# NoelShin/zutis

Hardware: AMD Instinct MI355X
Metric: images/sec, COCO2017-val-shaped ViT-B/16 dense semantic segmentation @336px (ZUTIS forward + semantic predict), batches of 32 per GPU, 3 independent batches in flight (higher is better)
Workload: dtype f16x3 (fp32-class)

## Files before the change

### include/zutis_hip.h

```cpp
#ifndef ZUTIS_HIP_H
#define ZUTIS_HIP_H

#include <stddef.h>

#ifdef __cplusplus
extern "C" {
#endif

typedef struct ihipStream_t* zh_stream_t;

#define ZH_OK 0
#define ZH_ERR_ARG (-1)
#define ZH_ERR_HIP (-2)
#define ZH_ERR_WORKSPACE (-3)

#define ZH_ACT_NONE 0
#define ZH_ACT_QUICKGELU 1
#define ZH_ACT_RELU 2
#define ZH_ACT_SIGMOID 3
#define ZH_ACT_GELU_ERF 4

#define ZH_ABI_VERSION 232
int zh_version(void);
const char* zh_arch(void);
const char* zh_last_error(void);

int zh_dev_set_gemm_overrides(int group_m, int tile, int tile_small);

int zh_dev_set_gemm_persist(int workgroups);

int zh_gemm_f16(const void* A, long lda, long strideA, const void* W, long ldw, long strideW,
                void* C, long ldc, long strideC, int out_f16,
                const float* bias, const float* residual, long ldr, long strideR, int res_rows,
                const void* pos_y, const void* pos_x, long ld_pos, int pos_h, int pos_w, int pos_f16,
                int act, int M, int N, int K, int batch, zh_stream_t stream);

int zh_gemm_f16_res16(const void* A, long lda, long strideA, const void* W, long ldw, long strideW,
// ... 41 lines not shown
                     const float* add, int add_rows, int rows, int D, long lo_plane, int* status, zh_stream_t stream);
#define ZH_STATUS_RANGE 1
#define ZH_STATUS_NONFINITE 2
#define ZH_STATUS_LABEL 4

int zh_sum_layernorm_f32(const float* parts, int n_parts, long part_stride, const float* bias, const float* residual,
                         float* out_sum, const float* gamma, const float* beta, float eps,
                         float* out_f32, void* out_f16, long lo_plane,
                         long out_group_rows, long out_group_stride, long out_offset, int skip_first_in_group,
                         const float* gamma2, const float* beta2, float eps2, float* out2_f32, void* out2_f16, long lo_plane2,
                         long out2_group_rows, long out2_group_stride, long out2_offset,
                         int rows, int D, int* status, zh_stream_t stream);

int zh_assemble_tokens_ln(const float* patch_emb, const float* class_embedding, const float* pos_embed,
                          const float* gamma, const float* beta, float eps, float* out,
                          int B, int T, int D, zh_stream_t stream);

int zh_assemble_tokens_ln_f16(const float* patch_emb, const float* class_embedding, const float* pos_embed,
                              const float* gamma, const float* beta, float eps, void* out,
                              int B, int T, int D, zh_stream_t stream);

int zh_l2norm_rows(const float* x, float* out_f32, void* out_f16, float eps, int rows, int D, long lo_plane, float f16_scale, zh_stream_t stream);

size_t zh_global_ln_l2_workspace_size(int B, int M, int C);
int zh_global_ln_l2(const float* x, float* out_f32, void* out_f16, float eps, float l2_eps,
                    int B, int M, int C, void* workspace, size_t workspace_bytes, long lo_plane, float f16_scale, int* status,
                    zh_stream_t stream);

int zh_im2col_f16(const float* x, void* out, int B, int Cin, int H, int W, int patch, int Kpad, int pad_to_patch,
                  long lo_plane, zh_stream_t stream);

int zh_posembed_bicubic(const float* pos, float* out, int grid, int h, int w, int D, float scale_h, float scale_w,
                        int has_cls, zh_stream_t stream);

int zh_upsample2x_bilinear_cl(const float* x, float* out_f32, void* out_f16, int B, int h, int w, int D, long lo_plane,
                              int relu, zh_stream_t stream);

int zh_sine_pe(float* out, int h, int w, int D, float temperature, zh_stream_t stream);

int zh_add_rowperiodic_f16(const void* a, const float* add, void* out, long rows, int D, int add_rows, long a_lo_plane,
                           long lo_plane, zh_stream_t stream);

// ... 136 lines not shown
```

### zutis_amd/csrc/common.h

```cpp
#pragma once
#include <hip/hip_runtime.h>
#include <stdint.h>
#include <stdio.h>

typedef _Float16 half_t;
typedef _Float16 half2_t __attribute__((ext_vector_type(2)));
typedef _Float16 half4_t __attribute__((ext_vector_type(4)));
typedef _Float16 half8_t __attribute__((ext_vector_type(8)));
typedef float f32x4 __attribute__((ext_vector_type(4)));
typedef float f32x16 __attribute__((ext_vector_type(16)));

#define ZH_OK 0
#define ZH_ERR_ARG (-1)
#define ZH_ERR_HIP (-2)
#define ZH_ERR_WORKSPACE (-3)

void zh_set_error(const char* fmt, ...);

#define ZH_CHECK_ARG(cond, ...)            \
  do {                                     \
    if (!(cond)) {                         \
      zh_set_error(__VA_ARGS__);           \
      return ZH_ERR_ARG;                   \
    }                                      \
// ... 55 lines not shown
  if (lo_plane) p[lo_plane] = (half_t)(y - (float)h);
}

struct LinW { int i0, i1; float l0, l1; };
__device__ __forceinline__ LinW lin_weights(int dst, int in_size, int out_size, float scale) {
  LinW r;
  if (in_size == out_size) { r.i0 = r.i1 = dst; r.l0 = 1.f; r.l1 = 0.f; return r; }
  const float src = fmaxf(__fmaf_rn(scale, (float)dst + 0.5f, -0.5f), 0.f);
  r.i0 = min((int)src, in_size - 1);
  r.i1 = min(r.i0 + 1, in_size - 1);
  r.l1 = fminf(fmaxf(src - (float)r.i0, 0.f), 1.f);
  r.l0 = 1.f - r.l1;
  return r;
}

#define ZH_ACT_NONE 0
#define ZH_ACT_QUICKGELU 1
#define ZH_ACT_RELU 2
#define ZH_ACT_SIGMOID 3
#define ZH_ACT_GELU_ERF 4

__device__ __forceinline__ float zh_act(float x, int act) {
  switch (act) {
    case ZH_ACT_QUICKGELU: return x * __builtin_amdgcn_rcpf(1.0f + __expf(-1.702f * x));
    case ZH_ACT_RELU: return fmaxf(x, 0.0f);
    case ZH_ACT_SIGMOID: return __builtin_amdgcn_rcpf(1.0f + __expf(-x));
    case ZH_ACT_GELU_ERF: return 0.5f * x * (1.0f + erff(x * 0.70710678118654752f));
    default: return x;
  }
}
// ... 1 lines not shown
```

### zutis_amd/csrc/norm.hip

```cpp
#include "common.h"

#define LN_MAXV 4

struct LnRow {
  f32x4 v[LN_MAXV];
};

#define ZH_STATUS_NONFINITE 2

__device__ __forceinline__ bool ln_normalize(LnRow& r, int nv, int lane, int D, float eps) {
  float s = 0.f;
#pragma unroll
  for (int j = 0; j < LN_MAXV; ++j)
    if (lane + 64 * j < nv) s += (r.v[j][0] + r.v[j][1]) + (r.v[j][2] + r.v[j][3]);
  const float mean = wave_sum(s) / (float)D;
  float q = 0.f;
#pragma unroll
  for (int j = 0; j < LN_MAXV; ++j)
    if (lane + 64 * j < nv) {
      r.v[j] -= mean;
      q += (r.v[j][0] * r.v[j][0] + r.v[j][1] * r.v[j][1]) + (r.v[j][2] * r.v[j][2] + r.v[j][3] * r.v[j][3]);
    }
  const float var = wave_sum(q) / (float)D;
  const float rstd = rsqrtf(var + eps);
// ... 186 lines not shown
  SumLnArgs p{parts, n_parts, part_stride, bias, residual, out_sum, gamma, beta, eps, out_f32, (half_t*)out_f16, lo_plane,
              out_group_rows, out_group_stride, out_offset, skip_first_in_group, gamma2, beta2, eps2, out2_f32, (half_t*)out2_f16, lo_plane2,
              out2_group_rows, out2_group_stride, out2_offset, rows, D, status};
  const dim3 grid(zh_cdiv(rows, 4));
  if (n_parts == 1) hipLaunchKernelGGL(sum_layernorm_kernel<1>, grid, dim3(256), 0, stream, p);
  else if (n_parts == 2) hipLaunchKernelGGL(sum_layernorm_kernel<2>, grid, dim3(256), 0, stream, p);
  else if (n_parts == 4) hipLaunchKernelGGL(sum_layernorm_kernel<4>, grid, dim3(256), 0, stream, p);
  else hipLaunchKernelGGL(sum_layernorm_kernel<0>, grid, dim3(256), 0, stream, p);
  ZH_CHECK_LAUNCH("zh_sum_layernorm_f32");
  return ZH_OK;
}

struct AsmArgs {
  const float* patch; const float* cls; const float* pos; const float* gamma; const float* beta;
  float* out; int B, T, D; float eps;
};

__global__ __launch_bounds__(256) void assemble_ln_kernel(AsmArgs p) {
  const int lane = threadIdx.x & 63;
  const long r = (long)blockIdx.x * 4 + (threadIdx.x >> 6);
  if (r >= (long)p.B * p.T) return;
  const int nv = p.D >> 2;
  const int b = (int)(r / p.T), t = (int)(r % p.T);
  const f32x4* src = t == 0 ? (const f32x4*)p.cls : (const f32x4*)(p.patch + ((long)b * (p.T - 1) + (t - 1)) * p.D);
  const f32x4* pos = (const f32x4*)(p.pos + (long)t * p.D);
  LnRow row;
#pragma unroll
  for (int j = 0; j < LN_MAXV; ++j)
    if (lane + 64 * j < nv) row.v[j] = src[lane + 64 * j] + pos[lane + 64 * j];
  if (p.gamma) ln_normalize(row, nv, lane, p.D, p.eps);
#pragma unroll
  for (int j = 0; j < LN_MAXV; ++j) {
    const int c = lane + 64 * j;
    if (c < nv) ((f32x4*)(p.out + r * p.D))[c] = p.gamma ? row.v[j] * ((const f32x4*)p.gamma)[c] + ((const f32x4*)p.beta)[c] : row.v[j];
  }
}

extern "C" int zh_assemble_tokens_ln(const float* patch_emb, const float* class_embedding, const float* pos_embed,
                                     const float* gamma, const float* beta, float eps, float* out,
                                     int B, int T, int D, hipStream_t stream) {
  ZH_CHECK_ARG(patch_emb && class_embedding && pos_embed && out, "zh_assemble_tokens_ln: null pointer");
  ZH_CHECK_ARG((gamma == nullptr) == (beta == nullptr), "zh_assemble_tokens_ln: gamma and beta must both be given or both null");
  ZH_CHECK_ARG(B > 0 && T > 1 && D % 4 == 0 && D <= 256 * LN_MAXV, "zh_assemble_tokens_ln: bad shape B=%d T=%d D=%d", B, T, D);
  AsmArgs p{patch_emb, class_embedding, pos_embed, gamma, beta, out, B, T, D, eps};
  hipLaunchKernelGGL(assemble_ln_kernel, dim3(zh_cdiv((long)B * T, 4)), dim3(256), 0, stream, p);
  ZH_CHECK_LAUNCH("zh_assemble_tokens_ln");
  return ZH_OK;
}

__device__ __forceinline__ bool ln_normalize_h8(LnRow& r, int nv8, int lane, int D, float eps) {
  float s = 0.f;
#pragma unroll
  for (int j = 0; j < LN_MAXV; ++j)
    if (lane + 64 * (j >> 1) < nv8) s += (r.v[j][0] + r.v[j][1]) + (r.v[j][2] + r.v[j][3]);
  const float mean = wave_sum(s) / (float)D;
  float q = 0.f;
#pragma unroll
  for (int j = 0; j < LN_MAXV; ++j)
    if (lane + 64 * (j >> 1) < nv8) {
// ... 88 lines not shown
  if (p.gamma) ln_normalize(row, nv, lane, p.D, p.eps);
  half_t* out = (half_t*)(void*)p.out + r * p.D;
#pragma unroll
  for (int j = 0; j < LN_MAXV; ++j) {
    const int c = lane + 64 * j;
    if (c < nv) zh_store_h4(out + 4 * c, 0, p.gamma ? row.v[j] * ((const f32x4*)p.gamma)[c] + ((const f32x4*)p.beta)[c] : row.v[j]);
  }
}

extern "C" int zh_assemble_tokens_ln_f16(const float* patch_emb, const float* class_embedding, const float* pos_embed,
                                         const float* gamma, const float* beta, float eps, void* out,
                                         int B, int T, int D, hipStream_t stream) {
  ZH_CHECK_ARG(patch_emb && class_embedding && pos_embed && out, "zh_assemble_tokens_ln_f16: null pointer");
  ZH_CHECK_ARG((gamma == nullptr) == (beta == nullptr), "zh_assemble_tokens_ln_f16: gamma and beta must both be given or both null");
  ZH_CHECK_ARG(B > 0 && T > 1 && D % 4 == 0 && D <= 256 * LN_MAXV, "zh_assemble_tokens_ln_f16: bad shape B=%d T=%d D=%d", B, T, D);
  AsmArgs p{patch_emb, class_embedding, pos_embed, gamma, beta, (float*)out, B, T, D, eps};
  hipLaunchKernelGGL(assemble_ln_h16_kernel, dim3(zh_cdiv((long)B * T, 4)), dim3(256), 0, stream, p);
  ZH_CHECK_LAUNCH("zh_assemble_tokens_ln_f16");
  return ZH_OK;
}

__global__ __launch_bounds__(256) void l2norm_rows_kernel(const float* x, float* out_f32, half_t* out_f16, int rows, int D, float eps,
                                                          long lo_plane, float f16_scale) {
  const int lane = threadIdx.x & 63;
  const long r = (long)blockIdx.x * 4 + (threadIdx.x >> 6);
  if (r >= rows) return;
  const int nv = D >> 2;
  const f32x4* xp = (const f32x4*)(x + r * D);
  f32x4 v[LN_MAXV];
  float q = 0.f;
#pragma unroll
// ... 99 lines not shown
#pragma unroll
  for (int j = 0; j < LN_MAXV; ++j)
    if (lane + 64 * j < nv) {
      v[j] = (xp[lane + 64 * j] - fmean) * rstd;
      q += (v[j][0] * v[j][0] + v[j][1] * v[j][1]) + (v[j][2] * v[j][2] + v[j][3] * v[j][3]);
    }
  const float inv = 1.0f / (sqrtf(wave_sum(q)) + l2_eps);
  const long ob = (long)img * per_image + r * C;
#pragma unroll
  for (int j = 0; j < LN_MAXV; ++j) {
    const int c = lane + 64 * j;
    if (c < nv) {
      f32x4 y = v[j] * inv;
      if (out_f32) ((f32x4*)(out_f32 + ob))[c] = y;
      if (out_f16) zh_store_h4(out_f16 + ob + 4 * c, lo_plane, y * f16_scale);
    }
  }
}

extern "C" size_t zh_global_ln_l2_workspace_size(int B, int M, int C) {
  const long per_image = (long)M * C;
  return (size_t)B * zh_cdiv(per_image, GLN_CHUNK) * 4 * sizeof(float);
}

extern "C" int zh_global_ln_l2(const float* x, float* out_f32, void* out_f16, float eps, float l2_eps,
                               int B, int M, int C, void* workspace, size_t workspace_bytes, long lo_plane, float f16_scale, int* status,
                               hipStream_t stream) {
  ZH_CHECK_ARG(x && (out_f32 || out_f16) && B > 0 && M > 0 && lo_plane % 4 == 0 && f16_scale > 0.f, "zh_global_ln_l2: bad arguments");
  ZH_CHECK_ARG(C % 4 == 0 && C <= 256 * LN_MAXV && C > 0, "zh_global_ln_l2: C=%d unsupported", C);
  ZH_CHECK_ARG(B < 65536, "zh_global_ln_l2: batch too large");
  const long per_image = (long)M * C;
  const int nchunks = zh_cdiv(per_image, GLN_CHUNK);
  if (workspace_bytes < zh_global_ln_l2_workspace_size(B, M, C) || !workspace) {
    zh_set_error("zh_global_ln_l2: workspace too small (%zu < %zu)", workspace_bytes, zh_global_ln_l2_workspace_size(B, M, C));
    return ZH_ERR_WORKSPACE;
  }
  hipLaunchKernelGGL(gln_partial_kernel, dim3(nchunks, B), dim3(256), 0, stream, x, (float*)workspace, per_image, nchunks);
  hipLaunchKernelGGL(gln_apply_kernel, dim3(zh_cdiv(M, 4), B), dim3(256), 0, stream, x, (const float*)workspace, out_f32,
                     (half_t*)out_f16, per_image, nchunks, M, C, eps, l2_eps, lo_plane, f16_scale, status);
  ZH_CHECK_LAUNCH("zh_global_ln_l2");
  return ZH_OK;
}
```

### zutis_amd/csrc/resample.hip

```cpp
#include "common.h"

__global__ __launch_bounds__(128) void im2col_kernel(const float* x, half_t* out, int B, int Cin, int H, int W, int p,
                                                     int gh, int gw, int Kpad, int vec, long lo_plane) {
  const int row = blockIdx.x;
  const int px = row % gw;
  const int t = row / gw;
  const int py = t % gh, b = t / gh;
  const int pp = p * p, kreal = Cin * pp;
  half_t* orow = out + (long)row * Kpad;
  for (int k0 = threadIdx.x * 8; k0 < Kpad; k0 += 128 * 8) {
    half8_t o;
    if (vec && k0 + 8 <= kreal) {
      const int c = k0 / pp, ij = k0 - c * pp, i = ij / p, j = ij - i * p;
      const int yy = py * p + i, xx = px * p + j;
      if (yy < H && xx + 8 <= W) {
        const f32x4* src = (const f32x4*)(x + (((long)b * Cin + c) * H + yy) * W + xx);
        const f32x4 v0 = src[0], v1 = src[1];
        zh_store_h4(orow + k0, lo_plane, v0);
        zh_store_h4(orow + k0 + 4, lo_plane, v1);
        continue;
      }
    }
#pragma unroll
    for (int e = 0; e < 8; ++e) {
// ... 93 lines not shown
  const int ya = max(j, 0), yb = min(j + 1, h - 1), xa = max(k, 0), xc = min(k + 1, w - 1);
  const f32x4* xb = (const f32x4*)(x + (long)b * h * w * D);
  const f32x4* p00 = xb + (long)(ya * w + xa) * nv;
  const f32x4* p01 = xb + (long)(ya * w + xc) * nv;
  const f32x4* p10 = xb + (long)(yb * w + xa) * nv;
  const f32x4* p11 = xb + (long)(yb * w + xc) * nv;
  float ly1[2], lx1[2];
  long orow[2];
  int ocol[2];
  bool vy[2], vx[2];
#pragma unroll
  for (int s = 0; s < 2; ++s) {
    const int oy = 2 * j + 1 + s, ox = 2 * k + 1 + s;
    vy[s] = oy >= 0 && oy < 2 * h;
    vx[s] = ox >= 0 && ox < 2 * w;
    const float sy = fmaxf(__fmaf_rn(0.5f, (float)oy + 0.5f, -0.5f), 0.f), sx = fmaxf(__fmaf_rn(0.5f, (float)ox + 0.5f, -0.5f), 0.f);
    const int y0 = min((int)sy, h - 1), x0 = min((int)sx, w - 1);
    ly1[s] = fminf(fmaxf(sy - (float)y0, 0.f), 1.f);
    lx1[s] = fminf(fmaxf(sx - (float)x0, 0.f), 1.f);
    orow[s] = ((long)b * 2 * h + oy) * (2 * w);
    ocol[s] = ox;
  }
  for (int c = threadIdx.x; c < nv; c += blockDim.x) {
    const f32x4 v00 = p00[c], v01 = p01[c], v10 = p10[c], v11 = p11[c];
#pragma unroll
    for (int sy = 0; sy < 2; ++sy)
#pragma unroll
      for (int sx = 0; sx < 2; ++sx) {
        if (!(vy[sy] && vx[sx])) continue;
        const float lx0 = 1.f - lx1[sx], ly0 = 1.f - ly1[sy];
        f32x4 o;
#pragma unroll
        for (int e = 0; e < 4; ++e) {
          const float r0 = __fmaf_rn(v00[e], lx0, __fmul_rn(v01[e], lx1[sx]));
          const float r1 = __fmaf_rn(v10[e], lx0, __fmul_rn(v11[e], lx1[sx]));
          o[e] = __fmaf_rn(r0, ly0, __fmul_rn(r1, ly1[sy]));
          if (relu) o[e] = fmaxf(o[e], 0.0f);
        }
        const long oi = (orow[sy] + ocol[sx]) * nv + c;
        if (out_f32) ((f32x4*)out_f32)[oi] = o;
        if (out_f16) zh_store_h4(out_f16 + 4 * oi, lo_plane, o);
      }
  }
}

extern "C" int zh_upsample2x_bilinear_cl(const float* x, float* out_f32, void* out_f16, int B, int h, int w, int D, long lo_plane,
                                         int relu, hipStream_t stream) {
  ZH_CHECK_ARG(x && (out_f32 || out_f16) && B > 0 && h > 0 && w > 0 && D > 0 && D % 4 == 0 && lo_plane % 4 == 0,
               "zh_upsample2x_bilinear_cl: bad arguments");
  const long quads = (long)B * (h + 1) * (w + 1);
  ZH_CHECK_ARG(quads < (1L << 31), "zh_upsample2x_bilinear_cl: too many output quads");
// ... 530 lines not shown
```

### zutis_amd/engine.py

```python
from __future__ import annotations

import math
import weakref
from typing import Dict, Optional, Tuple

import numpy as np
import torch

from . import _lib, compose, ops
from ._lib import ZutisHipError
from .engine_base import (ALL_SITES, DECODER_SITES, ENCODER_SITES, HEAD_SITES, PRECISIONS, P_shape0, _EngineBase, _rup, f16, f32,
                          resolve_precision)
from .ops import Act


def _to_host(t: torch.Tensor, cache: Dict[int, torch.Tensor]) -> np.ndarray:
    n = t.numel()
    if cache is None:
        cache = {}
    buf = cache.get(n)
    if buf is None:
        while len(cache) >= 8:
            cache.pop(next(iter(cache)))
        buf = cache[n] = torch.empty((n,), dtype=torch.uint8, pin_memory=True)
    buf.copy_(t, non_blocking=True)
    torch.cuda.current_stream(t.device).synchronize()
    return buf.numpy()


class ZutisEngine(_EngineBase):

    def __init__(self, params: Dict[str, torch.Tensor], patch: int, dec_heads: int = 8, precision="exact"):
        self.params = params
        self.patch = patch
        self.D = params["encoder.class_embedding"].shape[0]
        self.heads = self.D // 64
        self.layers = 1 + max(int(k.split(".")[3]) for k in params if k.startswith("encoder.transformer.resblocks."))
        self.dec_layers = 1 + max(int(k.split(".")[2]) for k in params if k.startswith("decoder.layers."))
        self.dec_heads = dec_heads
        self.dec_dh = self.D // dec_heads
        self.Q = params["query_embed"].shape[0]
        self.E = params["encoder.proj"].shape[1]
        self.grid = int(math.isqrt(params["encoder.positional_embedding"].shape[0] - 1))
        if self.dec_dh not in (64, 96):
            raise ZutisHipError(f"decoder head_dim {self.dec_dh} unsupported by zh_attention_f16 (64 or 96)")
        self._init_base(precision)

    def _pack(self):
        key = self._version_key()
        if key == self._packed_key:
            return
        P, D, w = self.params, self.D, {}
        c32 = self._c32
        self._pack_clip_visual(w, P, "encoder.", D, self.layers, self.patch)
        for ffn in ("ffn1", "ffn2"):
            for j in range(3):
                if (ffn, j) == ("ffn1", 2):
                    continue
                w[f"{ffn}.{j}.w"], w[f"{ffn}.{j}.b"] = self._hw(P[f"{ffn}.layers.{j}.weight"], ffn), c32(P[f"{ffn}.layers.{j}.bias"])
        W2, b2 = P["ffn1.layers.2.weight"].detach(), P["ffn1.layers.2.bias"].detach()
        self.Fh = W2.shape[1]
# ... 65 lines not shown
        g1 = self._abuf("ffn2_h1", (RQ, Fh), self._x3("ffn2"))
        g2 = self._abuf("ffn2_h2", (RQ, Fh), self._x3("ffn2"))
        q32 = self._buf("q32", (RQ, D), f32)
        q16 = self._abuf("q16", (RQ, D), self._x3("mask"), unit_norm=True)
        self._gemm("ffn2", inter16, W_["ffn2.0.w"], g1, bias=W_["ffn2.0.b"], act=ops.ACT_RELU)
        self._gemm("ffn2", g1, W_["ffn2.1.w"], g2, bias=W_["ffn2.1.b"], act=ops.ACT_RELU)
        self._gemm("ffn2", g2, W_["ffn2.2.w"], q32, bias=W_["ffn2.2.b"])
        ops.l2norm_rows(q32, RQ, D, out_f16=q16)
        masks = torch.empty((B, L, Q, h2, w2), dtype=f32, device=x.device)
        qw = self._abuf("mask_q", (RQ, FX), self._x3("mask"))
        self._gemm("mask", q16, W_["mask_q.w"], qw)
        self._gemm("mask", qw, f2x, masks, act=ops.ACT_SIGMOID, M=L * Q, N=M, K=FX, lda=FX, ldw=FX, ldc=M,
                   batch=B, strideA=L * Q * FX, strideW=M * FX, strideC=L * Q * M)
        tsl = self._buf("textspace_lo", (B * h * w, self.E), f32)
        self._gemm("textproj", tok16, W_["projT"], tsl)
        ts = self._buf("textspace", (B * M, self.E), f32)
        ops.upsample2x_cl(tsl, B, h, w, self.E, out_f32=ts)
        pt = torch.empty((B, h2, w2, self.E), dtype=f32, device=x.device)
        ws = self._buf("gln_ws", (max(1, ops.global_ln_l2_workspace_size(B, M, self.E)),), torch.uint8)
        pt16 = self._abuf("pt16", (B * M, self.E), self._x3("logits"), unit_norm=True)
        ops.global_ln_l2(ts, B, M, self.E, out_f32=pt, out_f16=pt16, eps=1e-5, l2_eps=1e-7, workspace=ws, status=self.status_word())
        self._pt16_of = (weakref.ref(pt), pt._version)
        return {"mask_proposals": masks, "patch_tokens": pt}

    def forward_graphed(self, x: torch.Tensor) -> Dict[str, torch.Tensor]:
        key = tuple(x.shape)
        graphs = self._graphs
        g = graphs.get(key)
        if g is not None and g["weights"] is self._packed_key:
            graphs.move_to_end(key)
            if g["graph"] is None:
                return self.forward(x)
            g["x"].copy_(x)
            g["graph"].replay()
            out = {k: v.clone() for k, v in g["out"].items()}
            if self._version_key() == self._packed_key:
# ... 306 lines not shown
```

### zutis_amd/engine_base.py

```python
from __future__ import annotations

import collections

import math
import os
import weakref
from typing import Dict, Optional, Tuple

import numpy as np
import torch

from . import _lib, compose, ops
from ._lib import ZutisHipError

from .ops import Act


def P_shape0(w) -> int:
    return (w.hi if isinstance(w, Act) else w).shape[0]

f16, f32 = torch.float16, torch.float32

ENCODER_SITES = ("conv", "qkv", "attn", "out", "fc", "proj")
DECODER_SITES = ("dec_kv", "dec")
# ... 70 lines not shown

    def _init_base(self, precision="exact", allow_half: bool = False):
        self.x3_sites = resolve_precision(precision, allow_half)
        self.precision = precision if isinstance(precision, str) else "custom"
        self.half_stream = precision == HALF
        self._packed_key = None
        self._w: Dict[str, torch.Tensor] = {}
        self._geo: Dict[Tuple[int, int], Dict[str, torch.Tensor]] = {}
        self._graphs: "collections.OrderedDict" = collections.OrderedDict()
        self._bufs: Dict[Tuple, torch.Tensor] = {}
        self._pinned: Dict[int, torch.Tensor] = {}
        self._buf_gen = 0
        self._buf_const: Dict[str, torch.Tensor] = {}
        self._pt16_of = self._text16_of = None
        self._status = None

    def fork(self):
        import copy
        self._pack()
        e = copy.copy(self)
        e._bufs, e._buf_gen, e._buf_const = {}, 0, {}
        e._geo = dict(self._geo)
        e._graphs = collections.OrderedDict()
        e._pinned = {}
        e._pt16_of = e._text16_of = None
        e._status = None
        return e

    def status_word(self) -> torch.Tensor:
        if self._status is None:
# ... 121 lines not shown
            w[q + "out_w"], w[q + "out_b"] = hw(P[p + "attn.out_proj.weight"], "out"), c32(P[p + "attn.out_proj.bias"])
            w[q + "fc_w"], w[q + "fc_b"] = hw(P[p + "mlp.c_fc.weight"], "fc"), c32(P[p + "mlp.c_fc.bias"])
            w[q + "proj_w"], w[q + "proj_b"] = hw(P[p + "mlp.c_proj.weight"], "proj"), c32(P[p + "mlp.c_proj.bias"])
            for ln, ln2 in (("ln_1", "ln1"), ("ln_2", "ln2")):
                w[q + ln2 + ".w"], w[q + ln2 + ".b"] = c32(P[p + ln + ".weight"]), c32(P[p + ln + ".bias"])

    def _clip_trunk(self, x: torch.Tensor, pos: torch.Tensor, h: int, w: int):
        W_, D, p = self._w, self.D, self.patch
        B = x.shape[0]
        T, R = 1 + h * w, B * (1 + h * w)
        col = self._abuf("col", (B * h * w, self.Kc), self._x3("conv"))
        ops.im2col(x, col, p, self.Kc)
        pe32 = self._buf("patch_emb", (B * h * w, D), f32)
        self._gemm("conv", col, W_["conv"], pe32)
        X = self._buf("X", (R, D), f16 if self.half_stream else f32)
        ops.assemble_tokens_ln(pe32, W_["encoder.class_embedding"], pos, W_["encoder.ln_pre.weight"],
                               W_["encoder.ln_pre.bias"], 1e-5, X, B, T, D)
        self._vit_blocks(X, B, T, D, self.heads, self.layers, 1e-5, ops.ACT_QUICKGELU)
        return X

    def _vit_blocks(self, X, B, T, D, heads, n_layers, eps, act, causal=False):
        W_, R = self._w, B * T
        Fd = P_shape0(W_["enc.0.fc_w"])
        Y = self._abuf("Y16", (R, D), self._x3("qkv", "fc"))
        xa = self._x3("attn")
        QKV = self._abuf("QKV16", (R, 3 * D), xa)
        O = self._abuf("O16", (R, D), self._x3("out"))
        Hh = self._abuf("H16", (R, Fd), self._x3("proj"))
        q_, k_, v_ = QKV, QKV.view(QKV.hi[:, D:]), QKV.view(QKV.hi[:, 2 * D:])
        st = self.status_word()
        s_out, s_proj = self._splitk(R, D, D), self._splitk(R, D, Fd)
        sk = self._x3("out") and self._x3("proj") and (s_out > 1 or s_proj > 1)
        if X.dtype == f16 and (self._x3("out") or self._x3("proj")):
            raise ZutisHipError("an fp16 residual stream needs the fp16-operand out / proj GEMMs (precision \"half\")")
        parts = self._buf("sk_parts", (max(s_out, s_proj), R, D), f32) if sk else None

# ... 1 lines not shown
            K = A.hi.shape[-1]
            return self._gemm(site, A, Wt, parts, M=R, N=D, K=K // S, lda=K, ldw=K, ldc=D, batch=S, strideA=K // S, strideW=K // S, strideC=R * D)
        eks, ews = 1, None
        if not causal:
            per_image = heads * -(-T // 128)
            eks = max(1, min(8, 256 // per_image)) if B * per_image <= 128 else 1
            ktiles = -(-T // (32 if xa else 64))
            if eks == 1 and T >= 2048:
                eks = long_sequence_key_split(B * per_image, ktiles, D // heads, xa, B * T * D)
            while eks > 1 and (eks - 1) * -(-ktiles // eks) >= ktiles:
                eks -= 1
            if eks > 1:
                ews = self._buf("enc_attn_ws", (ops.attention_splitk_workspace_size(B, heads, T, D // heads, eks),), torch.uint8)
        for i in range(n_layers):
            pp = f"enc.{i}."
            if not (sk and s_proj > 1 and i > 0):
                ops.layernorm(X, W_[pp + "ln1.w"], W_[pp + "ln1.b"], eps, R, D, out_f16=Y, status=st)
            self._gemm("qkv", Y, W_[pp + "qkv_w"], QKV, bias=W_[pp + "qkv_b"])
            ops.attention(q_, k_, v_, O, batch=B, heads=heads, Tq=T, Tk=T, head_dim=D // heads,
                          ldq=3 * D, ldk=3 * D, ldv=3 * D, ldo=D, strideQ=T * 3 * D, strideK=T * 3 * D, strideV=T * 3 * D,
                          strideO=T * D, causal=causal, x3=xa, ksplit=eks, workspace=ews)
            if sk and s_out > 1:
                gemm_parts("out", O, W_[pp + "out_w"], s_out)
                ops.sum_layernorm(parts, s_out, R, D, bias=W_[pp + "out_b"], residual=X, out_sum=X, gamma=W_[pp + "ln2.w"], beta=W_[pp + "ln2.b"],
                                  eps=eps, out_f16=Y, status=st)
            else:
                self._gemm("out", O, W_[pp + "out_w"], X, bias=W_[pp + "out_b"], residual=X)
                ops.layernorm(X, W_[pp + "ln2.w"], W_[pp + "ln2.b"], eps, R, D, out_f16=Y, status=st)
            self._gemm("fc", Y, W_[pp + "fc_w"], Hh, bias=W_[pp + "fc_b"], act=act)
            if sk and s_proj > 1:
                gemm_parts("proj", Hh, W_[pp + "proj_w"], s_proj)
# ... 107 lines not shown
```

### zutis_amd/ops.py

```python
from __future__ import annotations

import math
from typing import Optional

import numpy as np
import torch

from . import _lib

ACT_NONE, ACT_QUICKGELU, ACT_RELU, ACT_SIGMOID, ACT_GELU_ERF = 0, 1, 2, 3, 4
f16, f32 = torch.float16, torch.float32


PROFILER = None


def _call(entry: str, *args):
    _lib.check(getattr(_lib.load(), entry)(*args), entry)


def _launch(name, work, entry: str, args):
    fn = getattr(_lib.load(), entry)
    _lib.check(fn(*args) if PROFILER is None else PROFILER(name, work, lambda: fn(*args)), entry)

# ... 241 lines not shown
                  out_f32=None, out_f16=None, out_group_rows=None, out_group_stride=None, out_offset=0, skip_first_in_group=False,
                  gamma2=None, beta2=None, eps2=1e-5, out2_f32=None, out2_f16=None, out2_group_rows=None, out2_group_stride=None, out2_offset=0,
                  status=None):
    part_stride = rows * D if part_stride is None else part_stride
    ogr = rows if out_group_rows is None else out_group_rows
    ogs = ogr if out_group_stride is None else out_group_stride
    ogr2 = rows if out2_group_rows is None else out2_group_rows
    ogs2 = ogr2 if out2_group_stride is None else out2_group_stride
    (out_f16, lo1), (out2_f16, lo2) = _hp(out_f16), _hp(out2_f16)
    _call("zh_sum_layernorm_f32", _p(parts), n_parts, part_stride, _p(bias), _p(residual), _p(out_sum), _p(gamma), _p(beta), float(eps),
          _p(out_f32), _p(out_f16), lo1, ogr, ogs, out_offset, int(skip_first_in_group),
          _p(gamma2), _p(beta2), float(eps2), _p(out2_f32), _p(out2_f16), lo2, ogr2, ogs2, out2_offset,
          rows, D, _p(status), _stream())


def assemble_tokens_ln(patch_emb, cls, pos, gamma, beta, eps, out, B, T, D):
    _call("zh_assemble_tokens_ln_f16" if out.dtype == f16 else "zh_assemble_tokens_ln", _p(patch_emb), _p(cls), _p(pos), _p(gamma), _p(beta),
          float(eps), _p(out), B, T, D, _stream())


def _f16_scale(a) -> float:
    return 1.0 / a.out_scale if isinstance(a, Act) else 1.0


def l2norm_rows(x, rows, D, out_f32=None, out_f16=None, eps=0.0):
    sc = _f16_scale(out_f16)
    out_f16, lo = _hp(out_f16)
    _call("zh_l2norm_rows", _p(x), _p(out_f32), _p(out_f16), float(eps), rows, D, lo, sc, _stream())


def global_ln_l2_workspace_size(B, M, Cc) -> int:
    return int(_lib.load(raw=True).zh_global_ln_l2_workspace_size(B, M, Cc))


def global_ln_l2(x, B, M, Cc, out_f32=None, out_f16=None, eps=1e-5, l2_eps=1e-7, workspace=None, status=None):
    need = global_ln_l2_workspace_size(B, M, Cc)
    if workspace is None or _nbytes(workspace) < need:
        workspace = torch.empty(need, dtype=torch.uint8, device=x.device)
    sc = _f16_scale(out_f16)
    out_f16, lo = _hp(out_f16)
    _call("zh_global_ln_l2", _p(x), _p(out_f32), _p(out_f16), float(eps), float(l2_eps), B, M, Cc, _p(workspace),
          _nbytes(workspace), lo, sc, _p(status), _stream())


def im2col(x, out, patch, Kpad, pad_to_patch=False):
    B, Cin, H, W = x.shape
    _chk(x, f32, "im2col x")
    out, lo = _hp(out)
    _call("zh_im2col_f16", _p(x), _p(out), B, Cin, H, W, patch, Kpad, int(pad_to_patch), lo, _stream())


def posembed_bicubic(pos, out, grid, h, w, D, scale_h, scale_w, has_cls=True):
    _call("zh_posembed_bicubic", _p(pos), _p(out), grid, h, w, D, float(np.float32(scale_h)), float(np.float32(scale_w)), int(has_cls), _stream())


def upsample2x_cl(x, B, h, w, D, out_f32=None, out_f16=None, relu=False):
# ... 464 lines not shown
```

Before: 3076.

## Fuse upsample into global LN+L2 and chain first-block LayerNorm into token assembly

Adds a kernel pair that recomputes the 2x bilinear upsample on the fly inside the global LayerNorm+L2 normalisation. The full-resolution fp32 textspace buffer is no longer written and read back. Separately, the token-assembly ln_pre kernel now also applies the first encoder block's ln1 and writes the f16 (hi/lo) operand, skipping one layernorm launch and one pass over X. The fused path recomputes the interpolation in both the partial-stats and apply passes, and it changes the reduction structure, which could slightly alter numerics.

```diff
diff --git a/include/zutis_hip.h b/include/zutis_hip.h
--- a/include/zutis_hip.h
+++ b/include/zutis_hip.h
@@ -20,7 +20,7 @@
 #define ZH_ACT_SIGMOID 3
 #define ZH_ACT_GELU_ERF 4
 
-#define ZH_ABI_VERSION 232
+#define ZH_ABI_VERSION 233
 int zh_version(void);
 const char* zh_arch(void);
 const char* zh_last_error(void);
@@ -92,6 +92,7 @@
 
 int zh_assemble_tokens_ln(const float* patch_emb, const float* class_embedding, const float* pos_embed,
                           const float* gamma, const float* beta, float eps, float* out,
+                          const float* gamma2, const float* beta2, float eps2, void* out2_f16, long lo_plane2, int* status,
                           int B, int T, int D, zh_stream_t stream);
 
 int zh_assemble_tokens_ln_f16(const float* patch_emb, const float* class_embedding, const float* pos_embed,
@@ -104,6 +105,10 @@
 int zh_global_ln_l2(const float* x, float* out_f32, void* out_f16, float eps, float l2_eps,
                     int B, int M, int C, void* workspace, size_t workspace_bytes, long lo_plane, float f16_scale, int* status,
                     zh_stream_t stream);
+
+int zh_upsample2x_global_ln_l2(const float* x_lo, float* out_f32, void* out_f16, float eps, float l2_eps,
+                               int B, int h, int w, int C, void* workspace, size_t workspace_bytes, long lo_plane, float f16_scale,
+                               int* status, zh_stream_t stream);
 
 int zh_im2col_f16(const float* x, void* out, int B, int Cin, int H, int W, int patch, int Kpad, int pad_to_patch,
                   long lo_plane, zh_stream_t stream);
diff --git a/zutis_amd/csrc/common.h b/zutis_amd/csrc/common.h
--- a/zutis_amd/csrc/common.h
+++ b/zutis_amd/csrc/common.h
@@ -93,6 +93,29 @@
   return r;
 }
 
+__device__ __forceinline__ float zh_up2_l1(int o, int n) {
+  const float s = fmaxf(__fmaf_rn(0.5f, (float)o + 0.5f, -0.5f), 0.f);
+  const int i0 = min((int)s, n - 1);
+  return fminf(fmaxf(s - (float)i0, 0.f), 1.f);
+}
+__device__ __forceinline__ void zh_up2_taps(int o, int n, int& ia, int& ib) {
+  const int q = (o - 1) >> 1;
+  ia = max(q, 0);
+  ib = min(q + 1, n - 1);
+}
+__device__ __forceinline__ float zh_up2_lerp1(float v00, float v01, float v10, float v11, float lx0, float lx1, float ly0, float ly1) {
+  const float r0 = __fmaf_rn(v00, lx0, __fmul_rn(v01, lx1));
+  const float r1 = __fmaf_rn(v10, lx0, __fmul_rn(v11, lx1));
+  return __fmaf_rn(r0, ly0, __fmul_rn(r1, ly1));
+}
+__device__ __forceinline__ f32x4 zh_up2_lerp(f32x4 v00, f32x4 v01, f32x4 v10, f32x4 v11, float lx1, float ly1) {
+  const float lx0 = 1.f - lx1, ly0 = 1.f - ly1;
+  f32x4 o;
+#pragma unroll
+  for (int e = 0; e < 4; ++e) o[e] = zh_up2_lerp1(v00[e], v01[e], v10[e], v11[e], lx0, lx1, ly0, ly1);
+  return o;
+}
+
 #define ZH_ACT_NONE 0
 #define ZH_ACT_QUICKGELU 1
 #define ZH_ACT_RELU 2
diff --git a/zutis_amd/csrc/norm.hip b/zutis_amd/csrc/norm.hip
--- a/zutis_amd/csrc/norm.hip
+++ b/zutis_amd/csrc/norm.hip
@@ -224,6 +224,7 @@
 struct AsmArgs {
   const float* patch; const float* cls; const float* pos; const float* gamma; const float* beta;
   float* out; int B, T, D; float eps;
+  const float* gamma2; const float* beta2; float eps2; half_t* out2_f16; long lo_plane2; int* status;
 };
 
 __global__ __launch_bounds__(256) void assemble_ln_kernel(AsmArgs p) {
@@ -242,17 +243,33 @@
 #pragma unroll
   for (int j = 0; j < LN_MAXV; ++j) {
     const int c = lane + 64 * j;
-    if (c < nv) ((f32x4*)(p.out + r * p.D))[c] = p.gamma ? row.v[j] * ((const f32x4*)p.gamma)[c] + ((const f32x4*)p.beta)[c] : row.v[j];
+    if (c < nv) {
+      if (p.gamma) row.v[j] = row.v[j] * ((const f32x4*)p.gamma)[c] + ((const f32x4*)p.beta)[c];
+      ((f32x4*)(p.out + r * p.D))[c] = row.v[j];
+    }
+  }
+  if (!p.gamma2) return;
+#pragma unroll
+  for (int j = 0; j < LN_MAXV; ++j) asm("" : "+v"(row.v[j]));
+  zh_raise_nonfinite(p.status, ln_normalize(row, nv, lane, p.D, p.eps2), lane);
+#pragma unroll
+  for (int j = 0; j < LN_MAXV; ++j) {
+    const int c = lane + 64 * j;
+    if (c < nv) zh_store_h4(p.out2_f16 + r * p.D + 4 * c, p.lo_plane2, row.v[j] * ((const f32x4*)p.gamma2)[c] + ((const f32x4*)p.beta2)[c]);
   }
 }
 
 extern "C" int zh_assemble_tokens_ln(const float* patch_emb, const float* class_embedding, const float* pos_embed,
                                      const float* gamma, const float* beta, float eps, float* out,
+                                     const float* gamma2, const float* beta2, float eps2, void* out2_f16, long lo_plane2, int* status,
                                      int B, int T, int D, hipStream_t stream) {
   ZH_CHECK_ARG(patch_emb && class_embedding && pos_embed && out, "zh_assemble_tokens_ln: null pointer");
   ZH_CHECK_ARG((gamma == nullptr) == (beta == nullptr), "zh_assemble_tokens_ln: gamma and beta must both be given or both null");
+  ZH_CHECK_ARG((gamma2 == nullptr) == (beta2 == nullptr) && (gamma2 == nullptr) == (out2_f16 == nullptr),
+               "zh_assemble_tokens_ln: gamma2, beta2 and out2_f16 must all be given or all null");
+  ZH_CHECK_ARG(lo_plane2 % 4 == 0, "zh_assemble_tokens_ln: lo_plane2 must be a multiple of 4 halves");
   ZH_CHECK_ARG(B > 0 && T > 1 && D % 4 == 0 && D <= 256 * LN_MAXV, "zh_assemble_tokens_ln: bad shape B=%d T=%d D=%d", B, T, D);
-  AsmArgs p{patch_emb, class_embedding, pos_embed, gamma, beta, out, B, T, D, eps};
+  AsmArgs p{patch_emb, class_embedding, pos_embed, gamma, beta, out, B, T, D, eps, gamma2, beta2, eps2, (half_t*)out2_f16, lo_plane2, status};
   hipLaunchKernelGGL(assemble_ln_kernel, dim3(zh_cdiv((long)B * T, 4)), dim3(256), 0, stream, p);
   ZH_CHECK_LAUNCH("zh_assemble_tokens_ln");
   return ZH_OK;
@@ -371,7 +388,7 @@
   ZH_CHECK_ARG(patch_emb && class_embedding && pos_embed && out, "zh_assemble_tokens_ln_f16: null pointer");
   ZH_CHECK_ARG((gamma == nullptr) == (beta == nullptr), "zh_assemble_tokens_ln_f16: gamma and beta must both be given or both null");
   ZH_CHECK_ARG(B > 0 && T > 1 && D % 4 == 0 && D <= 256 * LN_MAXV, "zh_assemble_tokens_ln_f16: bad shape B=%d T=%d D=%d", B, T, D);
-  AsmArgs p{patch_emb, class_embedding, pos_embed, gamma, beta, (float*)out, B, T, D, eps};
+  AsmArgs p{patch_emb, class_embedding, pos_embed, gamma, beta, (float*)out, B, T, D, eps, nullptr, nullptr, 0.f, nullptr, 0, nullptr};
   hipLaunchKernelGGL(assemble_ln_h16_kernel, dim3(zh_cdiv((long)B * T, 4)), dim3(256), 0, stream, p);
   ZH_CHECK_LAUNCH("zh_assemble_tokens_ln_f16");
   return ZH_OK;
@@ -501,6 +518,160 @@
       f32x4 y = v[j] * inv;
       if (out_f32) ((f32x4*)(out_f32 + ob))[c] = y;
       if (out_f16) zh_store_h4(out_f16 + ob + 4 * c, lo_plane, y * f16_scale);
+    }
+  }
+}
+
+__device__ __forceinline__ void gln_chunk_partial(const f32x4 (&v)[4], long n, float* o) {
+#pragma clang fp contract(off)
+  float s = 0.f;
+#pragma unroll
+  for (int j = 0; j < 4; ++j) {
+    const long e = ((long)threadIdx.x + 256 * j) * 4;
+    if (e < n) s += (v[j][0] + v[j][1]) + (v[j][2] + v[j][3]);
+  }
+  __shared__ float red[4];
+  __shared__ float bc;
+  s = wave_sum(s);
+  if ((threadIdx.x & 63) == 0) red[threadIdx.x >> 6] = s;
+  __syncthreads();
+  if (threadIdx.x == 0) bc = ((red[0] + red[1]) + (red[2] + red[3])) / (float)n;
+  __syncthreads();
+  const float mean = bc;
+  float q = 0.f;
+#pragma unroll
+  for (int j = 0; j < 4; ++j) {
+    const long e = ((long)threadIdx.x + 256 * j) * 4;
+    if (e < n) {
+      f32x4 d = v[j] - mean;
+      q += (d[0] * d[0] + d[1] * d[1]) + (d[2] * d[2] + d[3] * d[3]);
+    }
+  }
+  q = wave_sum(q);
+  __syncthreads();
+  if ((threadIdx.x & 63) == 0) red[threadIdx.x >> 6] = q;
+  __syncthreads();
+  if (threadIdx.x == 0) {
+    o[0] = (float)n; o[1] = mean; o[2] = (red[0] + red[1]) + (red[2] + red[3]); o[3] = 0.f;
+  }
+}
+
+__device__ __forceinline__ bool gln_combine(const float* pp, int nchunks, int lane, float eps, float& fmean, float& rstd) {
+#pragma clang fp contract(off)
+  double sn = 0.0, sm = 0.0;
+  for (int i = lane; i < nchunks; i += 64) { sn += pp[4 * i]; sm = fma((double)pp[4 * i], (double)pp[4 * i + 1], sm); }
+#pragma unroll
+  for (int o = 32; o > 0; o >>= 1) { sn += __shfl_xor(sn, o, 64); sm += __shfl_xor(sm, o, 64); }
+  const double mean = sm / sn;
+  double m2 = 0.0;
+  for (int i = lane; i < nchunks; i += 64) {
+    const double d = (double)pp[4 * i + 1] - mean;
+    m2 += fma((double)pp[4 * i] * d, d, (double)pp[4 * i + 2]);
+  }
+#pragma unroll
+  for (int o = 32; o > 0; o >>= 1) m2 += __shfl_xor(m2, o, 64);
+  fmean = (float)mean;
+  rstd = (float)(1.0 / sqrt(m2 / sn + (double)eps));
+  return m2 / sn < (double)INFINITY;
+}
+
+template <int MAXV>
+__device__ __forceinline__ void gln_emit_row(const f32x4 (&x)[MAXV], int nv, int lane, float fmean, float rstd, float l2_eps,
+                                             float* out_f32, half_t* out_f16, long ob, long lo_plane, float f16_scale) {
+#pragma clang fp contract(off)
+  f32x4 v[MAXV];
+  float q = 0.f;
+#pragma unroll
+  for (int j = 0; j < MAXV; ++j)
+    if (lane + 64 * j < nv) {
+      v[j] = (x[j] - fmean) * rstd;
+      q += (v[j][0] * v[j][0] + v[j][1] * v[j][1]) + (v[j][2] * v[j][2] + v[j][3] * v[j][3]);
+    }
+  const float inv = 1.0f / (sqrtf(wave_sum(q)) + l2_eps);
+#pragma unroll
+  for (int j = 0; j < MAXV; ++j) {
+    const int c = lane + 64 * j;
+    if (c < nv) {
+      f32x4 y = v[j] * inv;
+      if (out_f32) ((f32x4*)(out_f32 + ob))[c] = y;
+      if (out_f16) zh_store_h4(out_f16 + ob + 4 * c, lo_plane, y * f16_scale);
+    }
+  }
+}
+
+__global__ __launch_bounds__(256) void up2_gln_partial_kernel(const float* x_lo, float* part, int h, int w, int C, int nchunks) {
+  const int img = blockIdx.x, ch = blockIdx.y;
+  const int per_image = 4 * h * w * C;
+  const int base = ch * GLN_CHUNK;
+  const long n = per_image - base < GLN_CHUNK ? per_image - base : GLN_CHUNK;
+  const int nv = C >> 2;
+  const unsigned w2 = 2 * w;
+  const f32x4* xb = (const f32x4*)(x_lo + (long)img * h * w * C);
+  f32x4 v[4];
+#pragma unroll
+  for (int j = 0; j < 4; ++j) {
+    const int e = ((int)threadIdx.x + 256 * j) * 4;
+    if (e < n) {
+      const unsigned a = (unsigned)(base + e), pix = a / (unsigned)C, c = (a - pix * (unsigned)C) >> 2;
+      const int oy = (int)(pix / w2), ox = (int)(pix - (unsigned)oy * w2);
+      int ya, yb, xa, xc;
+      zh_up2_taps(oy, h, ya, yb);
+      zh_up2_taps(ox, w, xa, xc);
+      v[j] = zh_up2_lerp(xb[(long)(ya * w + xa) * nv + c], xb[(long)(ya * w + xc) * nv + c], xb[(long)(yb * w + xa) * nv + c],
+                         xb[(long)(yb * w + xc) * nv + c], zh_up2_l1(ox, w), zh_up2_l1(oy, h));
+      asm("" : "+v"(v[j]));
+    }
+  }
+  gln_chunk_partial(v, n, part + ((long)img * nchunks + ch) * 4);
+}
+
+template <int MAXV>
+__global__ __launch_bounds__(256) void up2_gln_apply_kernel(const float* x_lo, const float* part, float* out_f32, half_t* out_f16,
+                                                            int h, int w, int C, int nchunks, float eps, float l2_eps,
+                                                            long lo_plane, float f16_scale, int* status) {
+  const int img = blockIdx.x;
+  const int lane = threadIdx.x & 63;
+  float fmean, rstd;
+  const bool finite = gln_combine(part + (long)img * nchunks * 4, nchunks, lane, eps, fmean, rstd);
+  if (status && blockIdx.y == 0 && threadIdx.x == 0 && !finite) atomicOr(status, ZH_STATUS_NONFINITE);
+
+  const int qw = w + 1;
+  const int quad = blockIdx.y * 4 + (threadIdx.x >> 6);
+  if (quad >= (h + 1) * qw) return;
+  const int k = quad % qw - 1, j = quad / qw - 1;
+  const int ya = max(j, 0), yb = min(j + 1, h - 1), xa = max(k, 0), xc = min(k + 1, w - 1);
+  const int nv = C >> 2;
+  const f32x4* xb = (const f32x4*)(x_lo + (long)img * h * w * C);
+  const f32x4* p00 = xb + (long)(ya * w + xa) * nv;
+  const f32x4* p01 = xb + (long)(ya * w + xc) * nv;
+  const f32x4* p10 = xb + (long)(yb * w + xa) * nv;
+  const f32x4* p11 = xb + (long)(yb * w + xc) * nv;
+  f32x4 v00[MAXV], v01[MAXV], v10[MAXV], v11[MAXV];
+#pragma unroll
+  for (int i = 0; i < MAXV; ++i) {
+    const int c = lane + 64 * i;
+    if (c < nv) { v00[i] = p00[c]; v01[i] = p01[c]; v10[i] = p10[c]; v11[i] = p11[c]; }
+  }
+  const long per_image = 4L * h * w * C;
+#pragma unroll
+  for (int sy = 0; sy < 2; ++sy) {
+    const int oy = 2 * j + 1 + sy;
+    if (oy < 0 || oy >= 2 * h) continue;
+    const float ly1 = zh_up2_l1(oy, h);
+#pragma unroll
+    for (int sx = 0; sx < 2; ++sx) {
+      const int ox = 2 * k + 1 + sx;
+      if (ox < 0 || ox >= 2 * w) continue;
+      const float lx1 = zh_up2_l1(ox, w);
+      f32x4 x[MAXV];
+#pragma unroll
+      for (int i = 0; i < MAXV; ++i)
+        if (lane + 64 * i < nv) {
+          x[i] = zh_up2_lerp(v00[i], v01[i], v10[i], v11[i], lx1, ly1);
+          asm("" : "+v"(x[i]));
+        }
+      gln_emit_row<MAXV>(x, nv, lane, fmean, rstd, l2_eps, out_f32, out_f16, (long)img * per_image + ((long)oy * 2 * w + ox) * C, lo_plane,
+                         f16_scale);
     }
   }
 }
@@ -528,3 +699,30 @@
   ZH_CHECK_LAUNCH("zh_global_ln_l2");
   return ZH_OK;
 }
+
+extern "C" int zh_upsample2x_global_ln_l2(const float* x_lo, float* out_f32, void* out_f16, float eps, float l2_eps,
+                                          int B, int h, int w, int C, void* workspace, size_t workspace_bytes, long lo_plane, float f16_scale,
+                                          int* status, hipStream_t stream) {
+  ZH_CHECK_ARG(x_lo && (out_f32 || out_f16) && B > 0 && h > 0 && w > 0 && lo_plane % 4 == 0 && f16_scale > 0.f,
+               "zh_upsample2x_global_ln_l2: bad arguments");
+  ZH_CHECK_ARG(C % 4 == 0 && C <= 256 * LN_MAXV && C > 0, "zh_upsample2x_global_ln_l2: C=%d unsupported", C);
+  const long per_image = 4L * h * w * C;
+  const long qblocks = ((long)(h + 1) * (w + 1) + 3) / 4;
+  ZH_CHECK_ARG(per_image < (1L << 31) && per_image / GLN_CHUNK < 65535 && qblocks < 65536,
+               "zh_upsample2x_global_ln_l2: image too large (h=%d w=%d C=%d)", h, w, C);
+  const int M = 4 * h * w;
+  const int nchunks = zh_cdiv(per_image, GLN_CHUNK);
+  if (workspace_bytes < zh_global_ln_l2_workspace_size(B, M, C) || !workspace) {
+    zh_set_error("zh_upsample2x_global_ln_l2: workspace too small (%zu < %zu)", workspace_bytes, zh_global_ln_l2_workspace_size(B, M, C));
+    return ZH_ERR_WORKSPACE;
+  }
+  hipLaunchKernelGGL(up2_gln_partial_kernel, dim3(B, nchunks), dim3(256), 0, stream, x_lo, (float*)workspace, h, w, C, nchunks);
+  if (C <= 512)
+    hipLaunchKernelGGL(up2_gln_apply_kernel<2>, dim3(B, (unsigned)qblocks), dim3(256), 0, stream, x_lo, (const float*)workspace, out_f32,
+                       (half_t*)out_f16, h, w, C, nchunks, eps, l2_eps, lo_plane, f16_scale, status);
+  else
+    hipLaunchKernelGGL(up2_gln_apply_kernel<LN_MAXV>, dim3(B, (unsigned)qblocks), dim3(256), 0, stream, x_lo, (const float*)workspace, out_f32,
+                       (half_t*)out_f16, h, w, C, nchunks, eps, l2_eps, lo_plane, f16_scale, status);
+  ZH_CHECK_LAUNCH("zh_upsample2x_global_ln_l2");
+  return ZH_OK;
+}
diff --git a/zutis_amd/csrc/resample.hip b/zutis_amd/csrc/resample.hip
--- a/zutis_amd/csrc/resample.hip
+++ b/zutis_amd/csrc/resample.hip
@@ -131,10 +131,8 @@
     const int oy = 2 * j + 1 + s, ox = 2 * k + 1 + s;
     vy[s] = oy >= 0 && oy < 2 * h;
     vx[s] = ox >= 0 && ox < 2 * w;
-    const float sy = fmaxf(__fmaf_rn(0.5f, (float)oy + 0.5f, -0.5f), 0.f), sx = fmaxf(__fmaf_rn(0.5f, (float)ox + 0.5f, -0.5f), 0.f);
-    const int y0 = min((int)sy, h - 1), x0 = min((int)sx, w - 1);
-    ly1[s] = fminf(fmaxf(sy - (float)y0, 0.f), 1.f);
-    lx1[s] = fminf(fmaxf(sx - (float)x0, 0.f), 1.f);
+    ly1[s] = zh_up2_l1(oy, h);
+    lx1[s] = zh_up2_l1(ox, w);
     orow[s] = ((long)b * 2 * h + oy) * (2 * w);
     ocol[s] = ox;
   }
@@ -149,9 +147,7 @@
         f32x4 o;
 #pragma unroll
         for (int e = 0; e < 4; ++e) {
-          const float r0 = __fmaf_rn(v00[e], lx0, __fmul_rn(v01[e], lx1[sx]));
-          const float r1 = __fmaf_rn(v10[e], lx0, __fmul_rn(v11[e], lx1[sx]));
-          o[e] = __fmaf_rn(r0, ly0, __fmul_rn(r1, ly1[sy]));
+          o[e] = zh_up2_lerp1(v00[e], v01[e], v10[e], v11[e], lx0, lx1[sx], ly0, ly1[sy]);
           if (relu) o[e] = fmaxf(o[e], 0.0f);
         }
         const long oi = (orow[sy] + ocol[sx]) * nv + c;
diff --git a/zutis_amd/engine.py b/zutis_amd/engine.py
--- a/zutis_amd/engine.py
+++ b/zutis_amd/engine.py
@@ -30,7 +30,7 @@
 
 class ZutisEngine(_EngineBase):
 
-    def __init__(self, params: Dict[str, torch.Tensor], patch: int, dec_heads: int = 8, precision="exact"):
+    def __init__(self, params: Dict[str, torch.Tensor], patch: int, dec_heads: int = 8, precision="exact", _fuse: bool = True):
         self.params = params
         self.patch = patch
         self.D = params["encoder.class_embedding"].shape[0]
@@ -45,6 +45,7 @@
         if self.dec_dh not in (64, 96):
             raise ZutisHipError(f"decoder head_dim {self.dec_dh} unsupported by zh_attention_f16 (64 or 96)")
         self._init_base(precision)
+        self._fuse = bool(_fuse)
 
     def _pack(self):
         key = self._version_key()
@@ -140,12 +141,16 @@
                    batch=B, strideA=L * Q * FX, strideW=M * FX, strideC=L * Q * M)
         tsl = self._buf("textspace_lo", (B * h * w, self.E), f32)
         self._gemm("textproj", tok16, W_["projT"], tsl)
-        ts = self._buf("textspace", (B * M, self.E), f32)
-        ops.upsample2x_cl(tsl, B, h, w, self.E, out_f32=ts)
         pt = torch.empty((B, h2, w2, self.E), dtype=f32, device=x.device)
         ws = self._buf("gln_ws", (max(1, ops.global_ln_l2_workspace_size(B, M, self.E)),), torch.uint8)
         pt16 = self._abuf("pt16", (B * M, self.E), self._x3("logits"), unit_norm=True)
-        ops.global_ln_l2(ts, B, M, self.E, out_f32=pt, out_f16=pt16, eps=1e-5, l2_eps=1e-7, workspace=ws, status=self.status_word())
+        if self._fuse:
+            ops.upsample2x_global_ln_l2(tsl, B, h, w, self.E, out_f32=pt, out_f16=pt16, eps=1e-5, l2_eps=1e-7, workspace=ws,
+                                        status=self.status_word())
+        else:
+            ts = torch.empty((B * M, self.E), dtype=f32, device=x.device)
+            ops.upsample2x_cl(tsl, B, h, w, self.E, out_f32=ts)
+            ops.global_ln_l2(ts, B, M, self.E, out_f32=pt, out_f16=pt16, eps=1e-5, l2_eps=1e-7, workspace=ws, status=self.status_word())
         self._pt16_of = (weakref.ref(pt), pt._version)
         return {"mask_proposals": masks, "patch_tokens": pt}
 
diff --git a/zutis_amd/engine_base.py b/zutis_amd/engine_base.py
--- a/zutis_amd/engine_base.py
+++ b/zutis_amd/engine_base.py
@@ -108,6 +108,7 @@
         self._buf_const: Dict[str, torch.Tensor] = {}
         self._pt16_of = self._text16_of = None
         self._status = None
+        self._fuse = True
 
     def fork(self):
         import copy
@@ -259,12 +260,16 @@
         pe32 = self._buf("patch_emb", (B * h * w, D), f32)
         self._gemm("conv", col, W_["conv"], pe32)
         X = self._buf("X", (R, D), f16 if self.half_stream else f32)
+        chain = self._fuse and not self.half_stream
+        Y = self._abuf("Y16", (R, D), self._x3("qkv", "fc")) if chain else None
         ops.assemble_tokens_ln(pe32, W_["encoder.class_embedding"], pos, W_["encoder.ln_pre.weight"],
-                               W_["encoder.ln_pre.bias"], 1e-5, X, B, T, D)
-        self._vit_blocks(X, B, T, D, self.heads, self.layers, 1e-5, ops.ACT_QUICKGELU)
+                               W_["encoder.ln_pre.bias"], 1e-5, X, B, T, D,
+                               gamma2=W_["enc.0.ln1.w"] if chain else None, beta2=W_["enc.0.ln1.b"] if chain else None, eps2=1e-5,
+                               out2_f16=Y, status=self.status_word() if chain else None)
+        self._vit_blocks(X, B, T, D, self.heads, self.layers, 1e-5, ops.ACT_QUICKGELU, ln1_done=chain)
         return X
 
-    def _vit_blocks(self, X, B, T, D, heads, n_layers, eps, act, causal=False):
+    def _vit_blocks(self, X, B, T, D, heads, n_layers, eps, act, causal=False, ln1_done=False):
         W_, R = self._w, B * T
         Fd = P_shape0(W_["enc.0.fc_w"])
         Y = self._abuf("Y16", (R, D), self._x3("qkv", "fc"))
@@ -296,7 +301,7 @@
                 ews = self._buf("enc_attn_ws", (ops.attention_splitk_workspace_size(B, heads, T, D // heads, eks),), torch.uint8)
         for i in range(n_layers):
             pp = f"enc.{i}."
-            if not (sk and s_proj > 1 and i > 0):
+            if not (sk and s_proj > 1 and i > 0) and not (ln1_done and i == 0):
                 ops.layernorm(X, W_[pp + "ln1.w"], W_[pp + "ln1.b"], eps, R, D, out_f16=Y, status=st)
             self._gemm("qkv", Y, W_[pp + "qkv_w"], QKV, bias=W_[pp + "qkv_b"])
             ops.attention(q_, k_, v_, O, batch=B, heads=heads, Tq=T, Tk=T, head_dim=D // heads,
diff --git a/zutis_amd/ops.py b/zutis_amd/ops.py
--- a/zutis_amd/ops.py
+++ b/zutis_amd/ops.py
@@ -279,9 +279,15 @@
           rows, D, _p(status), _stream())
 
 
-def assemble_tokens_ln(patch_emb, cls, pos, gamma, beta, eps, out, B, T, D):
-    _call("zh_assemble_tokens_ln_f16" if out.dtype == f16 else "zh_assemble_tokens_ln", _p(patch_emb), _p(cls), _p(pos), _p(gamma), _p(beta),
-          float(eps), _p(out), B, T, D, _stream())
+def assemble_tokens_ln(patch_emb, cls, pos, gamma, beta, eps, out, B, T, D, *, gamma2=None, beta2=None, eps2=1e-5, out2_f16=None, status=None):
+    if out.dtype == f16:
+        if out2_f16 is not None or gamma2 is not None:
+            raise _lib.ZutisHipError("assemble_tokens_ln: the chained LayerNorm needs the fp32 residual stream")
+        _call("zh_assemble_tokens_ln_f16", _p(patch_emb), _p(cls), _p(pos), _p(gamma), _p(beta), float(eps), _p(out), B, T, D, _stream())
+        return
+    out2_f16, lo2 = _hp(out2_f16)
+    _call("zh_assemble_tokens_ln", _p(patch_emb), _p(cls), _p(pos), _p(gamma), _p(beta), float(eps), _p(out),
+          _p(gamma2), _p(beta2), float(eps2), _p(out2_f16), lo2, _p(status) if out2_f16 is not None else None, B, T, D, _stream())
 
 
 def _f16_scale(a) -> float:
@@ -305,6 +311,15 @@
     sc = _f16_scale(out_f16)
     out_f16, lo = _hp(out_f16)
     _call("zh_global_ln_l2", _p(x), _p(out_f32), _p(out_f16), float(eps), float(l2_eps), B, M, Cc, _p(workspace),
+          _nbytes(workspace), lo, sc, _p(status), _stream())
+
+
+def upsample2x_global_ln_l2(x_lo, B, h, w, Cc, out_f32=None, out_f16=None, eps=1e-5, l2_eps=1e-7, workspace=None, status=None):
+    if workspace is None:
+        workspace = torch.empty(max(1, global_ln_l2_workspace_size(B, 4 * h * w, Cc)), dtype=torch.uint8, device=x_lo.device)
+    sc = _f16_scale(out_f16)
+    out_f16, lo = _hp(out_f16)
+    _call("zh_upsample2x_global_ln_l2", _p(x_lo), _p(out_f32), _p(out_f16), float(eps), float(l2_eps), B, h, w, Cc, _p(workspace),
           _nbytes(workspace), lo, sc, _p(status), _stream())
 
 
```

Result: no change. 3092, median of 6 (+0.5%).
